# Benny44/QPALM

Hardware: AMD Instinct MI355X
Metric: QP solves/sec (batched random n=1000,m=2000); `value` = solve only, batch resident in HBM -- with qpalm_setup in the clock as the reference's run_time has it: `value_setup_plus_solve` (higher is better)
Workload: dtype f64

## Files before the change

### qpalm_amd/csrc/qpalm_capi.inc

```
#include <math.h>
#include <stdio.h>
#include <stdlib.h>
#include <string.h>
#include <sys/mman.h>

#include <algorithm>
#include <atomic>
#include <chrono>
#include <thread>
#include <string>
#include <vector>
#include <map>

#include "../../include/qpalm_gfx950.h"

#ifdef QP_TWO_INSTANCES
#define QP_INST(ns, kern) ns::kern
#else
#define QP_INST(ns, kern) kern
#define QP_T_SMALL QP_T
#define QP_LDS_SMALL 38912
#define QP_T_TINY QP_T
#define QP_LDS_TINY 22016
#define QP_TINY_PER_CU 7
// ... 57 lines not shown
  int lds_bytes;
  int max_slots;
  int update_rank_threshold;
  int narrow_rows;
  int place_panel_wave;
  int small_workgroups;
  int coop;
  int coop_workgroups;
  int coop_max_batch;
  int coop_rank_threshold;
  int queue_order;
  int coop_test_kill;
  int coop_graphs;
  int coop_updates;
  int sweep_ranks;
  int kkt_compact;
  int sequential_rank_sums;
  int linesearch_hbm;
  int sparse_gpw;
  int sparse_lds;
  int sparse_ordering;
  int sparse_factor;
  int sparse_coop;
  int sparse_kkt;
  int ld_align;
  void *mv_buf[5];
  size_t mv_cap[5];
};

enum { H_AP, H_AI, H_ATP, H_ATI, H_ATPERM, H_AINV, H_QP, H_QI, H_QFP, H_QFI, H_QFPERM, H_AX, H_QX, H_Q, H_BMIN, H_BMAX, H_COUNT };
// ... 44 lines not shown
  double *raw_bmax() { return raw_h.data() + (size_t)B * n + (size_t)B * m; }
  double *raw_d_q() const { return (double *)raw_d; }
  double *raw_d_bmin() const { return (double *)raw_d + (size_t)B * n; }
  double *raw_d_bmax() const { return (double *)raw_d + (size_t)B * n + (size_t)B * m; }
};
static void co_graphs_clear(qpg_batch *bt) {
  for (auto &g : bt->co_graphs) if (g.second.ready) RT_GRAPH_FREE(g.second.exec);
  bt->co_graphs.clear();
}

extern "C" int qpg_ctx_create(int device, qpg_ctx **out) {
  if (!out) return fail(QPG_ERR_INVALID, "qpg_ctx_create: out is NULL");
  std::string why;
  if (RT_DEVICE_INIT(device, why) != 0) return fail(QPG_ERR_NO_DEVICE, "qpg_ctx_create: " + why);
  qpg_ctx *c = new qpg_ctx();
  c->device = device; c->lds_bytes = QPG_LDS_DEFAULT; c->max_slots = 512; c->update_rank_threshold = -1; c->small_workgroups = 1; c->place_panel_wave = 0; c->narrow_rows = 1; c->coop = -1; c->coop_workgroups = 256; c->coop_max_batch = 4; c->coop_rank_threshold = -2; c->coop_updates = 2; c->coop_test_kill = 0; c->queue_order = 1; c->coop_graphs = 1; c->ld_align = 16; c->sweep_ranks = 16; c->kkt_compact = 1; c->sparse_factor = -1; c->sparse_kkt = 0; c->sparse_coop = 0; c->sparse_ordering = -1; c->sparse_lds = 1; c->sparse_gpw = 0; c->linesearch_hbm = 0; c->sequential_rank_sums = -1;
  for (int k = 0; k < 5; k++) { c->mv_buf[k] = nullptr; c->mv_cap[k] = 0; }
  *out = c;
  return api_ok();
}
extern "C" void qpg_ctx_destroy(qpg_ctx *ctx) {
  if (!ctx) return;
  for (int k = 0; k < 5; k++) if (ctx->mv_buf[k]) RT_FREE(ctx->mv_buf[k]);
  RT_RELEASE_STREAMS();
  delete ctx;
}
static int ctx_scratch(qpg_ctx *ctx, int k, size_t bytes, void **p) {
  if (bytes > ctx->mv_cap[k]) {
    if (ctx->mv_buf[k]) RT_FREE(ctx->mv_buf[k]);
    ctx->mv_buf[k] = nullptr; ctx->mv_cap[k] = 0;
    const size_t cap = align_up(bytes + bytes / 2, 4096);
// ... 7 lines not shown
  if (!ctx || !name) return fail(QPG_ERR_INVALID, "qpg_ctx_set_option: NULL");
  if (!strcmp(name, "lds_bytes")) { if (value < QPG_LDS_DEFAULT || value > 160 * 1024 - 8192) return fail(QPG_ERR_INVALID, "lds_bytes out of range"); ctx->lds_bytes = (int)value; }
  else if (!strcmp(name, "max_slots")) { if (value < 1) return fail(QPG_ERR_INVALID, "max_slots < 1"); ctx->max_slots = (int)value; }
  else if (!strcmp(name, "update_rank_threshold")) ctx->update_rank_threshold = (int)value;
  else if (!strcmp(name, "small_workgroups")) ctx->small_workgroups = (value >= 0 && value <= 3) ? (int)value : 1;
  else if (!strcmp(name, "place_panel_wave")) ctx->place_panel_wave = (value < 0 || value > 2) ? 2 : (int)value;
  else if (!strcmp(name, "narrow_rows")) ctx->narrow_rows = value ? 1 : 0;
  else if (!strcmp(name, "coop")) ctx->coop = (value < 0) ? -1 : (value ? 1 : 0);
  else if (!strcmp(name, "coop_rank_threshold")) ctx->coop_rank_threshold = (value < -1) ? -2 : (int)value;
  else if (!strcmp(name, "coop_updates")) ctx->coop_updates = (value >= 0 && value <= 2) ? (int)value : 2;
  else if (!strcmp(name, "coop_graphs")) ctx->coop_graphs = value ? 1 : 0;
  else if (!strcmp(name, "coop_test_kill")) ctx->coop_test_kill = (int)value;
  else if (!strcmp(name, "queue_order")) ctx->queue_order = value ? 1 : 0;
  else if (!strcmp(name, "sweep_ranks")) { if (value != 16 && value != 32) return fail(QPG_ERR_INVALID, "sweep_ranks must be 16 or 32"); ctx->sweep_ranks = (int)value; }
  else if (!strcmp(name, "kkt_compact")) ctx->kkt_compact = value ? 1 : 0;
  else if (!strcmp(name, "sparse_factor")) ctx->sparse_factor = (value < 0) ? -1 : (value ? 1 : 0);
  else if (!strcmp(name, "sparse_kkt")) ctx->sparse_kkt = value ? 1 : 0;
  else if (!strcmp(name, "sparse_coop")) { if (value != 0 && value != 1) return fail(QPG_ERR_INVALID, "sparse_coop must be 0 or 1"); ctx->sparse_coop = (int)value; }
  else if (!strcmp(name, "sequential_rank_sums")) ctx->sequential_rank_sums = (value < 0) ? -1 : (value ? 1 : 0);
  else if (!strcmp(name, "linesearch_hbm")) ctx->linesearch_hbm = (value < 0) ? 0 : (int)std::min<qpg_int>(value, 1 << 20);
  else if (!strcmp(name, "sparse_gpw")) ctx->sparse_gpw = (int)value;
  else if (!strcmp(name, "sparse_lds")) ctx->sparse_lds = (value < 0) ? 0 : (int)value;
  else if (!strcmp(name, "sparse_ordering")) ctx->sparse_ordering = (value < 0) ? -1 : (value ? 1 : 0);
  else if (!strcmp(name, "ld_align")) { if (value != 8 && value != 16 && value != 32) return fail(QPG_ERR_INVALID, "ld_align must be 8, 16 or 32"); ctx->ld_align = (int)value; }
  else if (!strcmp(name, "coop_max_batch")) { if (value < 1) return fail(QPG_ERR_INVALID, "coop_max_batch < 1"); ctx->coop_max_batch = (int)value; }
  else if (!strcmp(name, "coop_workgroups")) { if (value < 1 || value > 4096) return fail(QPG_ERR_INVALID, "coop_workgroups out of range"); ctx->coop_workgroups = (int)value; }
  else return fail(QPG_ERR_INVALID, std::string("unknown option ") + name);
  return api_ok();
}

// ... 731 lines not shown
  bt->raw_h.clear(); bt->raw_cur = 0;
  bt->val_maps_current = false;
  V.B = bt->B; V.n = bt->n; V.m = bt->m; V.ld = bt->ld; V.nnzA = bt->nnzA; V.nnzQ = bt->nnzQ; V.nnzQf = bt->nnzQf;
  V.ls_hbm = bt->ctx->linesearch_hbm; V.seq_mode = bt->ctx->sequential_rank_sums;
  V.nslots = bt->nslots; V.lds_bytes = bt->lds_bytes; V.update_rank_threshold = bt->ctx->update_rank_threshold; V.place_panel_wave = bt->ctx->place_panel_wave;
  V.ls_stride = bt->ls_stride;
  {
    size_t nnz_rows = 0, rows = 0;
    for (auto &hp : bt->probs) { nnz_rows += (size_t)hp.nzA; rows += (size_t)hp.m; }
    const size_t colbufs = (size_t)4 * (bt->threads / 64) * bt->n * sizeof(double);
    V.narrow_rows = (bt->ctx->narrow_rows && !bt->kkt && colbufs <= (size_t)bt->lds_bytes && nnz_rows <= 16 * std::max<size_t>(rows, 1)) ? 1 : 0;
  }
  V.wst_stride = (int)QPG_WST_STRIDE(bt->nfac);
  V.sweep_ranks = bt->ctx->sweep_ranks;
  V.kkt_compact = bt->ctx->kkt_compact;
  V.kkt = bt->kkt; V.nfac = bt->nfac;
  if (ensure_dual_slots(bt) != 0) return fail(QPG_ERR_ALLOC, "device allocation failed (LD_Q slots)");
  V.sparse = 0; V.sp_co_G = 0; V.sp_co_wv = nullptr;
  bt->sp_plan.clear();
  if (bt->sparse) {
    const int rcs = sparse_setup(bt);
    if (rcs != QPG_OK) return rcs;
    if (ensure_dual_slots(bt) != 0) return fail(QPG_ERR_ALLOC, "device allocation failed (LD_Q values of the sparse factor)");
  }
  const size_t B = bt->B, n = bt->n, m = bt->m;
  {
    char *const dev[H_COUNT] = {(char *)V.Ap, (char *)V.Ai, (char *)V.Atp, (char *)V.Ati, (char *)V.Atperm, (char *)V.Ainv, (char *)V.Qp, (char *)V.Qi,
                                (char *)V.Qfp, (char *)V.Qfi, (char *)V.Qfperm, (char *)V.Ax, (char *)V.Qx, (char *)V.q, (char *)V.bmin, (char *)V.bmax};
    for (int a = 0; a < H_COUNT; a++)
      if (bt->hper[a] && RT_MEMCPY_H2D_ASYNC(dev[a], bt->hslab + bt->hoff[a], B * bt->hper[a] * bt->helem[a], 0) != 0)
// ... 924 lines not shown
```

### qpalm_amd/csrc/qpalm_dense.h

```cpp
#ifndef QPALM_DENSE_H
#define QPALM_DENSE_H
#include <type_traits>

#ifdef QPALM_EMU
#define QP_FLAG_LOAD(p) (*(volatile int *)(p))
#define QP_FLAG_STORE(p, v) (*(volatile int *)(p) = (v))
#define QP_RELEASE_AGENT() do { } while (0)
#define QP_ACQUIRE_AGENT() do { } while (0)
#define QP_DRAIN_VMEM() do { } while (0)
#define QP_SLEEP() do { } while (0)
#define QP_WAVE_SYNC() emu_wave_sync()
#define QP_LDS_VBASE(p) (p)
#define QP_SCHED_BARRIER() do { } while (0)
#define QP_SETPRIO(p) do { } while (0)
#define QP_DRAIN_LDS() do { } while (0)
#else
#define QP_FLAG_LOAD(p) __hip_atomic_load((p), __ATOMIC_RELAXED, __HIP_MEMORY_SCOPE_AGENT)
#define QP_FLAG_STORE(p, v) __hip_atomic_store((p), (v), __ATOMIC_RELAXED, __HIP_MEMORY_SCOPE_AGENT)
#define QP_RELEASE_AGENT() __builtin_amdgcn_fence(__ATOMIC_RELEASE, "agent")
#define QP_ACQUIRE_AGENT() __builtin_amdgcn_fence(__ATOMIC_ACQUIRE, "agent")
#define QP_DRAIN_VMEM() asm volatile("s_waitcnt vmcnt(0)" ::: "memory")
#define QP_SLEEP() __builtin_amdgcn_s_sleep(2)
#define QP_SETPRIO(p) __builtin_amdgcn_s_setprio(p)
#define QP_DRAIN_LDS() asm volatile("s_waitcnt lgkmcnt(0)" ::: "memory")
// ... 265 lines not shown
};

#ifndef QP_NI_FGEMM
#define QP_NI_FGEMM QPNI
#endif
#ifndef QP_FKC
#define QP_FKC 32
#endif
#define QP_FAS 66
#ifndef QP_FST
#define QP_FST 4
#endif
struct FactorStage { double As[2][QP_FKC][QP_FAS]; };

template <int NTJ, int NCT>
QP_NI_FGEMM void factor_panel_update(double *L_, const double *Dg_, char *stage_, int n_, int ld_, int J_, int tbase_, int k0_, int k1_) {
  const int n = QP_UNIFORM(n_), ld = QP_UNIFORM(ld_), J = QP_UNIFORM(J_), tbase = QP_UNIFORM(tbase_), k0 = QP_UNIFORM(k0_), k1 = QP_UNIFORM(k1_);
  qp_gdouble *L = (qp_gdouble *)L_;
  const qp_gdouble *Dg = (const qp_gdouble *)Dg_;
  FactorStage QP_LDS_AS &F = *QP_LDS_ARG(FactorStage, stage_);
  const int tid = threadIdx.x, lane = tid & 63, wid = tid >> 6;
  const int l15 = lane & 15, l4 = lane >> 4;
  constexpr bool PAIR = (NTJ == 2);
  constexpr int NBW = 16 * NCT;
  const int rbase = (J / 16 + tbase) * 16 + wid * 16 * NTJ;
  auto rowof = [&](const int t, const int j) QP_ALWAYS_INLINE { return PAIR ? (rbase + 2 * j + t) : (rbase + j); };
  auto colof = [&](const int ct, const int i) QP_ALWAYS_INLINE { return J + NCT * i + ct; };
  qp_double4 acc[NTJ][NCT];
  const bool full = QP_UNIFORM((int)((rbase >= J + NBW) && (rbase + 16 * NTJ <= n) && (J + NBW <= n))) != 0;
  if (full) {
#pragma unroll
    for (int ct = 0; ct < NCT; ct++)
#pragma unroll
      for (int r = 0; r < 4; r++) {
        double v[NTJ];
        qp_load_rows<NTJ>(L + (size_t)colof(ct, l4 + 4 * r) * ld + rowof(0, l15), v);
// ... 82 lines not shown
    for (int t = 0; t < NTJ; t++) {
      const int row = rowof(t, l15);
      if (row < n) {
#pragma unroll
        for (int ct = 0; ct < NCT; ct++)
#pragma unroll
          for (int r = 0; r < 4; r++) {
            const int col = colof(ct, l4 + 4 * r);
            if (col < n && row >= col) L[(size_t)col * ld + row] = acc[t][ct][r];
          }
      }
    }
  }
}

#ifndef QP_NI_FROWS
#define QP_NI_FROWS QPNI
#endif
QP_NI_FROWS void factor_panel_rows(double *L_, char *lds_, const int n_, const int ld_, const int J_, const int jb_) {
  const int n = QP_UNIFORM(n_), ld = QP_UNIFORM(ld_), J = QP_UNIFORM(J_), jb = QP_UNIFORM(jb_);
  qp_gdouble *L = (qp_gdouble *)L_;
  FactorLds QP_LDS_AS &F = *QP_LDS_ARG(FactorLds, lds_);
  constexpr int NB = QP_FNB;
  auto rows = [&](auto full) QP_ALWAYS_INLINE {
    constexpr bool FULL = decltype(full)::value;
#pragma unroll 1
    for (int i = J + jb + threadIdx.x; i < n; i += QP_T) {
      qp_gdouble *base = L + (size_t)J * ld + i;
      double u[NB];
#pragma unroll
      for (int c = 0; c < NB; c++) u[c] = (FULL || c < jb) ? base[(size_t)c * ld] : 0.0;
#pragma unroll
      for (int c = 0; c < NB; c++) {
        if (FULL || c < jb) {
          double v = u[c];
#pragma unroll
          for (int c1 = 0; c1 < c; c1++) {
            v = QP_FMA(-u[c1], F.Ld[c][c1], v);
            if ((c1 & 7) == 7) QP_SCHED_BARRIER();
          }
          u[c] = v;
        }
        QP_SCHED_BARRIER();
      }
      int ld2 = ld;
      QP_OPAQUE(ld2);
#pragma unroll
      for (int c = 0; c < NB; c++)
        if (FULL || c < jb) base[(size_t)c * ld2] = u[c] * F.dv[c];
    }
  };
  if (jb == NB) rows(std::true_type()); else rows(std::false_type());
}

#ifndef QP_NI_FDIAG
#define QP_NI_FDIAG QPNI
#endif
QP_NI_FDIAG void factor_diag_block(char *lds_) {
  FactorLds QP_LDS_AS &F = *QP_LDS_ARG(FactorLds, lds_);
  constexpr int NB = QP_FNB;
  const int r = (int)(threadIdx.x & (NB - 1));
  double p[NB];
#pragma unroll
  for (int c = 0; c < NB; c++) p[c] = F.Ld[r][c];
#pragma unroll
  for (int c = 0; c < NB; c++) {
    const double dc = qp_readlane(p[c], c);
    const double lic = p[c] / dc;
#pragma unroll
    for (int c2 = c + 1; c2 < NB; c2++) {
      const double s = qp_readlane(p[c], c2);
      p[c2] = QP_FMA(-lic, s, p[c2]);
    }
    p[c] = lic;
    if (r == c && threadIdx.x < NB) { F.dv[c] = 1.0 / dc; F.dg[c] = dc; }
  }
  if (threadIdx.x < NB) {
#pragma unroll
    for (int c = 0; c < NB; c++) if (r > c) F.Ld[r][c] = p[c];
  }
}

template <int RPT>
#ifndef QP_NI_FACTOR
#define QP_NI_FACTOR QPNI
#endif
QP_NI_FACTOR void dense_factor(double *L_, double *Dg_, int n_, int ld_, char *lds_, int64_t *tdbg_) {
  const int n = QP_UNIFORM(n_), ld = QP_UNIFORM(ld_);
  int64_t QP_LDS_AS *tdbg = (int64_t QP_LDS_AS *)tdbg_;
  qp_gdouble *L = (qp_gdouble *)L_, *Dg = (qp_gdouble *)Dg_;
  FactorLds QP_LDS_AS &F = *QP_LDS_ARG(FactorLds, lds_);
  const int tid = threadIdx.x, lane = tid & 63, wid = tid >> 6;
  const int NB = QP_FNB;
  __syncthreads();
  long long tq0 = QP_CLOCK();
  for (int J = 0; J < n; J += NB) {
    const int jb = (n - J < NB) ? (n - J) : NB;
    {
      const bool super = (J % (2 * NB)) == 0;
      const int k0 = super ? 0 : J - NB, k1 = J;
      if (k1 > k0) {
        const int ntiles = (n - J + 15) / 16;
        char *stage = lds_ + ((sizeof(FactorLds) + 15) & ~(size_t)15);
        for (int tbase = 0; tbase < ntiles; tbase += QP_FNT * QP_NW) {
          const int rem = ntiles - tbase;
          const int ntj = (rem + QP_NW - 1) / QP_NW;
          if (super) {
            if (ntj <= 1) factor_panel_update<1, 4>(L_, Dg_, stage, n, ld, J, tbase, k0, k1);
            else factor_panel_update<2, 4>(L_, Dg_, stage, n, ld, J, tbase, k0, k1);
          } else {
            if (ntj <= 1) factor_panel_update<1, 2>(L_, Dg_, stage, n, ld, J, tbase, k0, k1);
            else factor_panel_update<2, 2>(L_, Dg_, stage, n, ld, J, tbase, k0, k1);
          }
        }
        if (tid == 0) {
          const long long npass = (ntiles + QP_FNT * QP_NW - 1) / (QP_FNT * QP_NW);
          tdbg[QPG_CNT_FACTOR_REREAD] += (long long)(n - J) * (k1 - k0) + npass * (super ? 2 * NB : NB) * (long long)(k1 - k0);
        }
      }
    }
    __syncthreads();
    if (tid == 0) { const long long tq1 = QP_CLOCK(); tdbg[4] += tq1 - tq0; tq0 = tq1; }
    for (int e = tid; e < NB * NB; e += QP_T) {
      const int c = e / NB, r = e % NB;
      F.Ld[r][c] = (r >= c && r < jb) ? L[(size_t)(J + c) * ld + (J + r)] : ((r == c) ? 1.0 : 0.0);
    }
    __syncthreads();
    if (wid == 0) factor_diag_block(lds_);
    __syncthreads();
    for (int e = tid; e < jb * jb; e += QP_T) {
      const int c = e / jb, r = e % jb;
      if (r > c) L[(size_t)(J + c) * ld + (J + r)] = F.Ld[r][c];
    }
    if (tid < jb) Dg[J + tid] = F.dg[tid];
    if (tid == 0) { const long long tq1 = QP_CLOCK(); tdbg[5] += tq1 - tq0; tq0 = tq1; }
    factor_panel_rows(L_, lds_, n, ld, J, jb);
    __syncthreads();
    if (tid == 0) { const long long tq1 = QP_CLOCK(); tdbg[6] += tq1 - tq0; tq0 = tq1; }
  }
  __syncthreads();
}

#define QP_SNB 32
#ifndef QP_SOLVE_FCH
#define QP_SOLVE_FCH 16
#endif
#ifndef QP_SOLVE_BU
#define QP_SOLVE_BU 4
#endif
struct SolveLds {
  double tile[2][QP_SNB][QP_SNB + 1];
  double part[QP_SNB];
};

// ... 1347 lines not shown
```

### qpalm_amd/csrc/qpalm_device.h

```cpp
#ifndef QPALM_DEVICE_H
#define QPALM_DEVICE_H

#include "qpalm_types.h"

#ifndef QP_T
#define QP_T 512
#endif
#define QP_NW (QP_T / 64)
#ifndef QP_KSEL
#define QP_KSEL(RPT) ((RPT) <= 2 ? 16 : 8)
#endif
#ifndef QP_K32
#ifdef QPALM_EMU
#define QP_K32(RPT) ((RPT) >= 1 && (RPT) <= 2)
#define QP_LDS_BUDGET QPG_LDS_DEFAULT
#else
#define QP_K32(RPT) (QP_T >= 512 && (RPT) >= 1 && (RPT) <= 2)
#define QP_LDS_BUDGET ((QP_T >= 512) ? QPG_LDS_DEFAULT : 38912)
#endif
#endif
#define QPD __device__ __forceinline__
#define QPN __device__ __forceinline__
#ifndef QP_PHASE_CALLS
#define QP_PHASE_CALLS 2
// ... 30 lines not shown
#endif

#ifdef QPALM_EMU
typedef emu_double4 qp_double4;
#define QP_MFMA_F64(a, b, c) emu_mfma_f64_16x16x4((a), (b), (c))
#define QP_DYN_LDS() (emu::dyn_lds())
#define QP_FMA(a, b, c) std::fma((a), (b), (c))
#define QP_SQRT(x) std::sqrt(x)
#define QP_CLOCK() ((long long)wall_clock64())
#define QP_UNIFORM(x) (x)
#define QP_UNIFORM_PTR(p) (p)
#define QP_OPAQUE(x) do { } while (0)
#define QP_OPAQUE_V(x) do { } while (0)
#define QP_FRESH_LANE(lane) (lane)
#define QP_CALL_BLOCK() 1
#define QP_ALWAYS_INLINE
#define QP_HW_CU_KEY() 0
#define QP_HW_SIMD() ((int)(threadIdx.x >> 6) & 3)
#else
typedef double qp_double4 __attribute__((ext_vector_type(4)));
#define QP_MFMA_F64(a, b, c) __builtin_amdgcn_mfma_f64_16x16x4f64((a), (b), (c), 0, 0, 0)
extern __shared__ __attribute__((aligned(16))) char qp_dyn_lds_[];
static __device__ __forceinline__ char *qp_dyn_lds_opaque_() {
  unsigned a = (unsigned)(size_t)(char __attribute__((address_space(3))) *)qp_dyn_lds_;
  asm volatile("" : "+s"(a));
  return (char *)(char __attribute__((address_space(3))) *)(size_t)a;
}
#define QP_DYN_LDS() (qp_dyn_lds_opaque_())
#define QP_FMA(a, b, c) fma((a), (b), (c))
#define QP_SQRT(x) sqrt(x)
// ... 1 lines not shown
#define QP_UNIFORM(x) __builtin_amdgcn_readfirstlane(x)
template <class P> static __device__ __forceinline__ P qp_uniform_ptr_(P p) {
  const unsigned long long a = (unsigned long long)p;
  const unsigned lo = (unsigned)__builtin_amdgcn_readfirstlane((int)(unsigned)a), hi = (unsigned)__builtin_amdgcn_readfirstlane((int)(unsigned)(a >> 32));
  return (P)(((unsigned long long)hi << 32) | lo);
}
#define QP_UNIFORM_PTR(p) qp_uniform_ptr_(p)
#define QP_OPAQUE(x) do { (x) = __builtin_amdgcn_readfirstlane(x); asm volatile("" : "+s"(x)); } while (0)
#define QP_OPAQUE_V(x) asm volatile("" : "+v"(x))
static __device__ __forceinline__ int qp_fresh_lane_() {
  int z = 0;
  asm volatile("s_mov_b32 %0, 0" : "=s"(z));
  return (int)__builtin_amdgcn_mbcnt_hi(~0u, __builtin_amdgcn_mbcnt_lo(~0u, (unsigned)z));
}
#define QP_FRESH_LANE(lane) qp_fresh_lane_()
static __device__ __forceinline__ int qp_opaque_true_() {
  int one;
  asm volatile("s_mov_b32 %0, 1" : "=s"(one));
  return one;
}
#define QP_CALL_BLOCK() qp_opaque_true_()
#define QP_ALWAYS_INLINE __attribute__((always_inline))
#define QP_HW_SIMD() ((int)__builtin_amdgcn_s_getreg((2 - 1) << 11 | 4 << 6 | 4))
#define QP_HW_CU_KEY() ((int)(__builtin_amdgcn_s_getreg((8 - 1) << 11 | 8 << 6 | 4) | (__builtin_amdgcn_s_getreg((4 - 1) << 11 | 0 << 6 | 20) << 8)))
#endif

QPD double qmax(double a, double b) { return (a > b) ? a : b; }
QPD double qmin(double a, double b) { return (a < b) ? a : b; }
QPD double qabs(double x) { return (x < 0) ? -x : x; }

// ... 191 lines not shown
```

### qpalm_amd/csrc/qpalm_iter.h

```cpp
#ifndef QPALM_ITER_H
#define QPALM_ITER_H
#ifndef QP_NOFUSE
#define QP_NOFUSE 0
#endif

#define QP_KIND_NEWTON 0
#define QP_KIND_OUTER 1
#define QP_KIND_FORCED 2
#define QP_KIND_TERMINATED 3

QPD int qp_prox(const qpg_settings &st, const qpg_scalars &s) { return (st.proximal != 0 || s.nc_flag != 0) ? 1 : 0; }
QPD double qp_gamma_init(const qpg_settings &st, const qpg_scalars &s) { return s.nc_flag ? s.nc_gamma : st.gamma_init; }
QPD double qp_gamma_max(const qpg_settings &st, const qpg_scalars &s) { return s.nc_flag ? s.nc_gamma : st.gamma_max; }

struct IterShared {
  QpShared S;
  qpg_scalars s;
  int kind, action, nL, pos;
  double a0, b0;
  double scan_a[QP_NW], scan_b[QP_NW];
};

struct QpArrays {
  const qpg_view *V; int b, n, m;
// ... 187 lines not shown
    vs[2] += t * t;
  }
  block_reduce<0, 3>(I.S, vm, vs);
  const double f = 0.5 * vs[0] + vs[1], dist2 = vs[2];
  const double sig = qmax(1e-4, qmin(st.sigma_init * qmax(1, qabs(f)) / qmax(1, 0.5 * dist2), 1e4));
  const double ssig = QP_SQRT(sig), sinv = 1.0 / sig;
  for (int i = tid; i < m; i += QP_T) {
    a.sigma()[i] = sig; a.sigma_inv()[i] = sinv; a.sqrt_sigma()[i] = ssig; a.At_scale()[i] = ssig;
    for (int k = a.Atp()[i]; k < a.Atp()[i + 1]; k++) a.Atss()[k] = a.Atx()[k] * ssig;
  }
  if (tid == 0) { I.s.sqrt_sigma_max = QP_SQRT(st.sigma_max); I.s.initialized = 1; }
  __syncthreads();
}

template <int RPT>
QPN void dev_factor(const qpg_view &V, int n, double *L, double *Dg, char *lds, int64_t *tdbg) { dense_factor<RPT>(L, Dg, n, V.ld, lds, tdbg); }
template <int RPT>
QPN void dev_updown(const qpg_view &V, int b, int n, double *L, double *Dg, double *Wst, const int *up, int n_up,
                    const int *dn, int n_dn, QpShared &S, char *lds, int64_t *tdbg, double *fs = nullptr, int pre_jmin = -1) {
  const int *Atp = V.Atp + (size_t)b * (V.m + 1), *Ati = V.Ati + (size_t)b * V.nnzA;
  const double *Atss = V.Atss + (size_t)b * V.nnzA;
  __syncthreads();
  if (threadIdx.x == 0) S.seq_ranks = qp_pivot_mode(V, b);
  __syncthreads();
  if constexpr (RPT == 0) dense_updown_big<16>(Atp, Ati, Atss, n, V.ld, L, Dg, Wst, up, n_up, dn, n_dn, &S, lds, tdbg, pre_jmin);
  else if constexpr (QP_K32(RPT)) {
    const int nr = n_up + n_dn;
    int n32 = 0;
    if (V.sweep_ranks >= 32 && pre_jmin < 0 && nr > 16) n32 = (nr % 32 > 16 || nr % 32 == 0) ? nr : nr - nr % 32;
    if (n32 > 0) dense_updown<1, 32>(Atp, Ati, Atss, n, V.ld, L, Dg, Wst, up, n_up, dn, n_dn, &S, lds, tdbg, -1, (n32 == nr) ? fs : nullptr, 0, n32);
    if (n32 < nr) dense_updown<RPT, QP_KSEL(RPT)>(Atp, Ati, Atss, n, V.ld, L, Dg, Wst, up, n_up, dn, n_dn, &S, lds, tdbg, pre_jmin, fs, n32, nr - n32);
// ... 663 lines not shown
    }
    if (V.offload && !resume && !V.kkt && (la == 1 || la == 3 || la == 7 || (kind == QP_KIND_NEWTON && la == 0) || (V.offload >= 2 && (la == 2 || la == 4)))) {
      if (kind == QP_KIND_NEWTON && la != 7) {
        for (int j = tid; j < n; j += QP_T) a.d()[j] = a.dphi()[j] * -1;
      }
      __syncthreads();
      if (tid == 0) {
        I.s.pend_stage = 1; I.s.pend_la = (la == 1 || la == 3 || la == 7 || la == 2 || la == 4) ? la : 0; I.s.pend_action = action; I.s.pend_kind = kind;
        I.s.pend_nchange = (la == 4) ? n_sig : nchange; I.s.pend_gam = gam;
      }
      __syncthreads();
      break;
    }
    const long long t0 = QP_CLOCK();
    double gersh_ub = 0.0;
    if constexpr (SPARSE) {
      const SpArrays SP = sp_arrays(V, b, slot, Dg, lds);
      if (resume) {
        if (la == 7) {
          SpArrays SQ = SP; SQ.Lx = LQ; SQ.Dg = DgQ;
          const double dobj = dev_dual_objective_sp(V, a, b, SQ, I);
          if (tid == 0) { I.s.dual_objective = dobj; I.s.dual_pending = 0; }
          __syncthreads();
          continue;
        }
      } else
      if (la == 2) {
        sp_updown(V, b, n, SP, a.enter(), I.s.nb_enter, a.leave(), I.s.nb_leave);
        if (V.offload && kind == QP_KIND_NEWTON) {
          for (int j = tid; j < n; j += QP_T) a.d()[j] = a.dphi()[j] * -1;
// ... 16 lines not shown
        continue;
      }
    } else
    if (resume) {
      if (la == 7) {
        const double dobj = dev_dual_objective(V, a, b, LQ, DgQ, I, lds);
        if (tid == 0) { I.s.dual_objective = dobj; I.s.dual_pending = 0; }
        __syncthreads();
        continue;
      }
    } else
    if (la == 1 || la == 3 || la == 5 || la == 7) {
      double *Lt = (la == 7) ? LQ : L, *Dt = (la == 7) ? DgQ : Dg;
      gersh_ub = form_schur(V, b, n, Lt, la == 5, la == 1 || la == 5, (la == 1 || la == 3) && (prox != 0), gam, I.S, lds);
      if (tid == 0) I.s.ticks_dbg[3] += QP_CLOCK() - t0;
      if (la != 5) dev_factor<RPT>(V, n, Lt, Dt, lds, I.s.ticks_dbg);
      if (dual_init) {
        const double dobj = dev_dual_objective(V, a, b, LQ, DgQ, I, lds);
        if (tid == 0) { I.s.dual_objective = dobj; I.s.dual_pending = 0; }
        __syncthreads();
        continue;
      }
    } else if (la == 8) {
      kkt_newton<RPT>(&V, b, L, Dg, Wst, &I, lds, action, I.s.nb_enter, I.s.nb_leave, QP_KKT_SOLVE | QP_KKT_REFINE);
    } else if (la == 2 || la == 4) {
      const int n_up = (la == 2) ? I.s.nb_enter : n_sig, n_dn = (la == 2) ? I.s.nb_leave : 0;
      double *fs = nullptr;
      constexpr bool FUSED = (RPT > 0) && !QP_NOFUSE;
      if (FUSED && la == 2 && !V.offload) {
        for (int j = tid; j < n; j += QP_T) a.d()[j] = a.dphi()[j] * -1;
        fs = a.d();
// ... 10 lines not shown
    }
    const long long t1 = QP_CLOCK();
    QP_OPAQUE(a.b);
    if (la == 4) {
      dev_update_sigma_post(a, I, n_sig);
      if (tid == 0) { I.s.n_sweeps = (int)I.s.ticks_dbg[QPG_CNT_SWEEPS]; I.s.ticks_update += t1 - t0; }
    } else if (la == 5 || la == 6) dev_boost_gamma_apply(V, a, I, gersh_ub);
    if (kind == QP_KIND_NEWTON) {
      if constexpr (SPARSE) {
        if (!V.kkt && !resume) {
          for (int j = tid; j < n; j += QP_T) a.d()[j] = a.dphi()[j] * -1;
          sp_solve(n, sp_arrays(V, b, slot, Dg, lds), a.d());
        }
      } else
      if (!V.kkt && !resume) {
        const bool fused = (RPT > 0) && !QP_NOFUSE && (action == 2) && !V.offload;
        if (!fused) for (int j = tid; j < n; j += QP_T) a.d()[j] = a.dphi()[j] * -1;
        __syncthreads();
        dense_solve(L, Dg, n, V.ld, a.d(), lds, V.lds_bytes, I.s.ticks_dbg, fused ? 2 : 0);
      }
      const long long t2 = QP_CLOCK();
      for (int i = tid; i < m; i += QP_T) a.active_old()[i] = a.active()[i];
      if (tid == 0) {
        I.s.reset_newton = 0;
        I.s.kkt_first = 0;
        if (action == 1) { I.s.n_refactor++; I.s.ticks_factor += t1 - t0; }
        if (action == 3) { I.s.n_factor_Q++; I.s.ticks_factor += t1 - t0; }
        if (action == 2) { if (!V.kkt) I.s.n_rank1 += nchange; I.s.n_sweeps = (int)I.s.ticks_dbg[QPG_CNT_SWEEPS]; I.s.ticks_update += t1 - t0; }
        I.s.n_solve++; I.s.ticks_solve += t2 - t1;
        if (!V.kkt && (RPT > 0) && !QP_NOFUSE && action == 2 && (SPARSE || !V.offload)) I.s.n_fused_solve++;
        I.s.last_fact = action;
      }
      QP_OPAQUE(a.b);
      const double tau = dev_linesearch(V, a, I, lds);
      const long long t3 = QP_CLOCK();
      QP_OPAQUE(a.b);
      {
        const int gs = QP_UNIFORM(I.s.guard_spent);
        const double ge = I.s.eta, gb = I.s.beta;
        const bool bad = !(qabs(ge) <= 1.7976931348623157e308) || !(qabs(gb) <= 1.7976931348623157e308);
        const int what = ((action == 0 || action == 2 || gs == 2) && gs != 1 && bad) ? ((gs == 2) ? 2 : 1) : ((gs == 2) ? 3 : 0);
        const int w = QP_UNIFORM(what);
        if (w != 0) {
          __syncthreads();
          if (tid == 0) {
// ... 51 lines not shown
```

### qpalm_amd/csrc/qpalm_kkt.h

```cpp
#ifndef QPALM_KKT_H
#define QPALM_KKT_H

QPD void kkt_form(const qpg_view &V, const QpArrays &a, int b, double *L, double gamma, int prox) {
  const int n = a.n, m = a.m, np = n + m, ld = V.ld, tid = threadIdx.x;
  int *state = V.kkt_state + (size_t)b * V.m;
  __syncthreads();
  for (int j = 0; j < np; j++)
    for (int i = j + tid; i < np; i += QP_T) L[(size_t)j * ld + i] = 0.0;
  __syncthreads();
  for (int j = tid; j < n; j += QP_T) {
    for (int k = a.Qp()[j]; k < a.Qp()[j + 1]; k++) { const int i = a.Qi()[k]; if (i >= j) L[(size_t)j * ld + i] += a.Qx()[k]; }
    if (prox) L[(size_t)j * ld + j] += 1.0 / gamma;
  }
  for (int k = tid; k < m; k += QP_T) {
    const int p = n + k, e0 = a.Atp()[k], e1 = a.Atp()[k + 1];
    if (a.active()[k]) {
      state[k] = 1;
      for (int e = e0; e < e1; e++) L[(size_t)a.Ati()[e] * ld + p] = a.Atx()[e];
      L[(size_t)p * ld + p] = (e1 > e0) ? -a.sigma_inv()[k] : 1.0;
    } else { state[k] = 0; L[(size_t)p * ld + p] = 1.0; }
  }
  __syncthreads();
}

// ... 136 lines not shown
  const qpg_view &V = *Vp;
  IterShared &I = *Ip;
  const int b = QP_UNIFORM(b_), action = QP_UNIFORM(action_), ne = QP_UNIFORM(ne_), nl = QP_UNIFORM(nl_), flags = QP_UNIFORM(flags_);
  const QpArrays a = qp_arrays(V, b);
  const qpg_settings &st = *V.settings;
  const int n = a.n, m = a.m, np = n + m, ld = V.ld, tid = threadIdx.x, lane = tid & 63, wid = tid >> 6, prox = qp_prox(st, I.s);
  const double gamma = I.s.gamma;
  const size_t sk = (size_t)V.n + V.m;
  double *sol = V.kkt_sol + (size_t)b * sk, *rhs = V.kkt_rhs + (size_t)b * sk, *z = V.kkt_tmp + (size_t)b * sk;
  int *state = V.kkt_state + (size_t)b * V.m;
  int *list = V.kkt_list + (size_t)b * V.m;
  const bool can_compact = V.kkt_compact && ((size_t)QP_NW * np * sizeof(double) + (size_t)m * sizeof(int) <= (size_t)V.lds_bytes);
  int kna = QP_UNIFORM(I.s.kkt_na);
  if (action == 1 && can_compact) {
    kna = kkt_form_compact(V, a, b, L, gamma, prox, I, list);
    dense_factor<RPT>(L, Dg, n + kna, ld, lds, I.s.ticks_dbg);
  } else {
    if (kna >= 0 && (action == 2 || action == 5)) { kkt_expand(V, a, L, Dg, kna, list, lds); kna = -1; }
    if (action == 1 || action == 3) { kkt_form(V, a, b, L, gamma, prox); kna = -1; }
    if (action == 1 || action == 4) { dense_factor<RPT>(L, Dg, np, ld, lds, I.s.ticks_dbg); kna = -1; }
  }
  __syncthreads();
  if (tid == 0) I.s.kkt_na = kna;
  __syncthreads();
  if (action == 2) {
    for (int e = 0; e < ne + nl; e++) {
      const bool add = e < ne;
      const int k = QP_UNIFORM(add ? a.enter()[e] : a.leave()[e - ne]), p = n + k;
      __syncthreads();
      int up;
      if (add) {
        for (int j = tid; j < np; j += QP_T) z[j] = 0.0;
        __syncthreads();
        for (int q = a.Atp()[k] + tid; q < a.Atp()[k + 1]; q += QP_T) z[a.Ati()[q]] = a.Atx()[q];
        __syncthreads();
// ... 76 lines not shown
```

### qpalm_amd/csrc/qpalm_types.h

```cpp
#ifndef QPALM_TYPES_H_GFX950
#define QPALM_TYPES_H_GFX950

#include <stdint.h>

#define QPG_SOLVED 1
#define QPG_DUAL_TERMINATED 2
#define QPG_MAX_ITER_REACHED (-2)
#define QPG_PRIMAL_INFEASIBLE (-3)
#define QPG_DUAL_INFEASIBLE (-4)
#define QPG_TIME_LIMIT_REACHED (-5)
#define QPG_UNSOLVED (-10)
#define QPG_ERROR 0
#define QPG_INFTY 1e20

typedef struct {
  int64_t max_iter, inner_max_iter;
  double eps_abs, eps_rel, eps_abs_in, eps_rel_in, rho, eps_prim_inf, eps_dual_inf, theta, delta, sigma_max,
      sigma_init;
  int64_t proximal;
  double gamma_init, gamma_upd, gamma_max;
  int64_t scaling, nonconvex, verbose, print_iter, warm_start, reset_newton_iter, enable_dual_termination;
  double dual_objective_limit, time_limit;
  int64_t ordering, factorization_method, max_rank_update;
  double max_rank_update_fraction;
// ... 24 lines not shown
  int32_t pend_stage, pend_la, pend_action, pend_kind, pend_nchange;
  int32_t seq_hint;
  int32_t kkt_na;
  double pend_gam;
  int64_t pend_clock;
  int32_t guard_redo, n_guard_refactor, guard_spent, guard_pad;
  int32_t dual_pending, kkt_first;
  int32_t n_refactor, n_factor_Q, n_sweeps, n_rank1, n_solve, n_sigma_updates, n_boost_gamma, n_fused_solve;
  int64_t ticks_total, ticks_factor, ticks_update, ticks_solve, ticks_linesearch, ticks_resid;
  int64_t ticks_dbg[QPG_NDBG];
} qpg_scalars;

typedef struct {
  int32_t B, n, m, ld, nnzA, nnzQ, nnzQf, nslots, lds_bytes, update_rank_threshold, ls_stride, wst_stride, place_panel_wave, narrow_rows;
  int32_t offload, sweep_ranks;
  int32_t kkt_compact, kkt_pad;
  int32_t kkt, nfac;
  int32_t *Ap, *Ai, *Atp, *Ati, *Atperm, *Ainv, *Qp, *Qi, *Qfp, *Qfi, *Qfperm;
  double *Ax, *Atx, *Atss, *Qx, *Qfx;
  double *q, *bmin, *bmax, *c0;
  double *x, *y, *Axv, *Qxv, *Aty, *x_prev, *x0;
  double *sigma, *sigma_inv, *sqrt_sigma, *At_scale;
  double *Axys, *z, *pri_res, *pri_res_in, *yh, *Atyh, *df, *dphi, *dphi_prev, *d, *Qd, *Ad;
  double *delta_y, *delta_x, *temp_n, *temp_m;
  double *D, *Dinv, *E, *Einv;
  double *ls_key;
  int32_t *ls_idx;
  double *ls_delta, *ls_alpha;
  int32_t *active, *active_old, *enter, *leave;
  double *sol_x, *sol_y;
  double *L;
// ... 43 lines not shown
```

Measured before the change: 5363.

## Fuse forward substitution into dense LDL factorization for Newton refactors

During a full dense factorization in the Newton step, the right-hand side is kept in LDS and the forward triangular solve is done alongside the factorization. The diagonal block applies its unit-lower solve to the panel's entries, and the panel-row pass updates the remaining entries as L columns are produced. The later dense_solve then skips its forward phase, which saves one extra pass over L in HBM. This costs extra LDS for an n-length vector, adds a fit check, and inlines previously noinline helpers, which may change register pressure.

```diff
diff --git a/qpalm_amd/csrc/qpalm_capi.inc b/qpalm_amd/csrc/qpalm_capi.inc
--- a/qpalm_amd/csrc/qpalm_capi.inc
+++ b/qpalm_amd/csrc/qpalm_capi.inc
@@ -95,6 +95,7 @@
   int coop_graphs;
   int coop_updates;
   int sweep_ranks;
+  int factor_fused_solve;
   int kkt_compact;
   int sequential_rank_sums;
   int linesearch_hbm;
@@ -169,7 +170,7 @@
   std::string why;
   if (RT_DEVICE_INIT(device, why) != 0) return fail(QPG_ERR_NO_DEVICE, "qpg_ctx_create: " + why);
   qpg_ctx *c = new qpg_ctx();
-  c->device = device; c->lds_bytes = QPG_LDS_DEFAULT; c->max_slots = 512; c->update_rank_threshold = -1; c->small_workgroups = 1; c->place_panel_wave = 0; c->narrow_rows = 1; c->coop = -1; c->coop_workgroups = 256; c->coop_max_batch = 4; c->coop_rank_threshold = -2; c->coop_updates = 2; c->coop_test_kill = 0; c->queue_order = 1; c->coop_graphs = 1; c->ld_align = 16; c->sweep_ranks = 16; c->kkt_compact = 1; c->sparse_factor = -1; c->sparse_kkt = 0; c->sparse_coop = 0; c->sparse_ordering = -1; c->sparse_lds = 1; c->sparse_gpw = 0; c->linesearch_hbm = 0; c->sequential_rank_sums = -1;
+  c->device = device; c->lds_bytes = QPG_LDS_DEFAULT; c->max_slots = 512; c->update_rank_threshold = -1; c->small_workgroups = 1; c->place_panel_wave = 0; c->narrow_rows = 1; c->coop = -1; c->coop_workgroups = 256; c->coop_max_batch = 4; c->coop_rank_threshold = -2; c->coop_updates = 2; c->coop_test_kill = 0; c->queue_order = 1; c->coop_graphs = 1; c->ld_align = 16; c->sweep_ranks = 16; c->kkt_compact = 1; c->factor_fused_solve = 1; c->sparse_factor = -1; c->sparse_kkt = 0; c->sparse_coop = 0; c->sparse_ordering = -1; c->sparse_lds = 1; c->sparse_gpw = 0; c->linesearch_hbm = 0; c->sequential_rank_sums = -1;
   for (int k = 0; k < 5; k++) { c->mv_buf[k] = nullptr; c->mv_cap[k] = 0; }
   *out = c;
   return api_ok();
@@ -207,6 +208,7 @@
   else if (!strcmp(name, "queue_order")) ctx->queue_order = value ? 1 : 0;
   else if (!strcmp(name, "sweep_ranks")) { if (value != 16 && value != 32) return fail(QPG_ERR_INVALID, "sweep_ranks must be 16 or 32"); ctx->sweep_ranks = (int)value; }
   else if (!strcmp(name, "kkt_compact")) ctx->kkt_compact = value ? 1 : 0;
+  else if (!strcmp(name, "factor_fused_solve")) ctx->factor_fused_solve = value ? 1 : 0;
   else if (!strcmp(name, "sparse_factor")) ctx->sparse_factor = (value < 0) ? -1 : (value ? 1 : 0);
   else if (!strcmp(name, "sparse_kkt")) ctx->sparse_kkt = value ? 1 : 0;
   else if (!strcmp(name, "sparse_coop")) { if (value != 0 && value != 1) return fail(QPG_ERR_INVALID, "sparse_coop must be 0 or 1"); ctx->sparse_coop = (int)value; }
@@ -968,6 +970,7 @@
   V.wst_stride = (int)QPG_WST_STRIDE(bt->nfac);
   V.sweep_ranks = bt->ctx->sweep_ranks;
   V.kkt_compact = bt->ctx->kkt_compact;
+  V.factor_fused_solve = bt->ctx->factor_fused_solve;
   V.kkt = bt->kkt; V.nfac = bt->nfac;
   if (ensure_dual_slots(bt) != 0) return fail(QPG_ERR_ALLOC, "device allocation failed (LD_Q slots)");
   V.sparse = 0; V.sp_co_G = 0; V.sp_co_wv = nullptr;
diff --git a/qpalm_amd/csrc/qpalm_dense.h b/qpalm_amd/csrc/qpalm_dense.h
--- a/qpalm_amd/csrc/qpalm_dense.h
+++ b/qpalm_amd/csrc/qpalm_dense.h
@@ -303,12 +303,12 @@
 struct FactorStage { double As[2][QP_FKC][QP_FAS]; };
 
 template <int NTJ, int NCT>
-QP_NI_FGEMM void factor_panel_update(double *L_, const double *Dg_, char *stage_, int n_, int ld_, int J_, int tbase_, int k0_, int k1_) {
+QPD void factor_panel_update_body(double *L_, const double *Dg_, char *stage_, int n_, int ld_, int J_, int tbase_, int k0_, int k1_) {
   const int n = QP_UNIFORM(n_), ld = QP_UNIFORM(ld_), J = QP_UNIFORM(J_), tbase = QP_UNIFORM(tbase_), k0 = QP_UNIFORM(k0_), k1 = QP_UNIFORM(k1_);
   qp_gdouble *L = (qp_gdouble *)L_;
   const qp_gdouble *Dg = (const qp_gdouble *)Dg_;
   FactorStage QP_LDS_AS &F = *QP_LDS_ARG(FactorStage, stage_);
-  const int tid = threadIdx.x, lane = tid & 63, wid = tid >> 6;
+  const int tid = QP_FRESH_TID(), lane = tid & 63, wid = tid >> 6;
   const int l15 = lane & 15, l4 = lane >> 4;
   constexpr bool PAIR = (NTJ == 2);
   constexpr int NBW = 16 * NCT;
@@ -421,18 +421,27 @@
   }
 }
 
+#define QP_FACTOR_YS_OFF (((sizeof(FactorLds) + 15) & ~(size_t)15) + sizeof(FactorStage))
+QPD bool factor_solve_fits(const int n, const int lds_bytes) { return QP_FACTOR_YS_OFF + (size_t)n * sizeof(double) <= (size_t)lds_bytes; }
+
+template <int NTJ, int NCT>
+QP_NI_FGEMM void factor_panel_update(double *L_, const double *Dg_, char *stage_, int n_, int ld_, int J_, int tbase_, int k0_, int k1_) {
+  factor_panel_update_body<NTJ, NCT>(L_, Dg_, stage_, n_, ld_, J_, tbase_, k0_, k1_);
+}
+
 #ifndef QP_NI_FROWS
-#define QP_NI_FROWS QPNI
-#endif
-QP_NI_FROWS void factor_panel_rows(double *L_, char *lds_, const int n_, const int ld_, const int J_, const int jb_) {
+#define QP_NI_FROWS QPD
+#endif
+QP_NI_FROWS void factor_panel_rows(double *L_, char *lds_, const int n_, const int ld_, const int J_, const int jb_, const int fuse_ = 0) {
   const int n = QP_UNIFORM(n_), ld = QP_UNIFORM(ld_), J = QP_UNIFORM(J_), jb = QP_UNIFORM(jb_);
   qp_gdouble *L = (qp_gdouble *)L_;
   FactorLds QP_LDS_AS &F = *QP_LDS_ARG(FactorLds, lds_);
+  double QP_LDS_AS *ys = QP_LDS_ARG(double, lds_ + QP_FACTOR_YS_OFF);
   constexpr int NB = QP_FNB;
-  auto rows = [&](auto full) QP_ALWAYS_INLINE {
-    constexpr bool FULL = decltype(full)::value;
+  auto rows = [&](auto full, auto fused) QP_ALWAYS_INLINE {
+    constexpr bool FULL = decltype(full)::value, FUSE = decltype(fused)::value;
 #pragma unroll 1
-    for (int i = J + jb + threadIdx.x; i < n; i += QP_T) {
+    for (int i = J + jb + QP_FRESH_TID(); i < n; i += QP_T) {
       qp_gdouble *base = L + (size_t)J * ld + i;
       double u[NB];
 #pragma unroll
@@ -452,21 +461,34 @@
       }
       int ld2 = ld;
       QP_OPAQUE(ld2);
-#pragma unroll
-      for (int c = 0; c < NB; c++)
-        if (FULL || c < jb) base[(size_t)c * ld2] = u[c] * F.dv[c];
+      if (FUSE) {
+        double acc = ys[i];
+#pragma unroll
+        for (int c = 0; c < NB; c++)
+          if (FULL || c < jb) {
+            const double l = u[c] * F.dv[c];
+            base[(size_t)c * ld2] = l;
+            acc = QP_FMA(-l, ys[J + c], acc);
+          }
+        ys[i] = acc;
+      } else {
+#pragma unroll
+        for (int c = 0; c < NB; c++)
+          if (FULL || c < jb) base[(size_t)c * ld2] = u[c] * F.dv[c];
+      }
     }
   };
-  if (jb == NB) rows(std::true_type()); else rows(std::false_type());
+  if (QP_UNIFORM(fuse_) != 0) { if (jb == NB) rows(std::true_type(), std::true_type()); else rows(std::false_type(), std::true_type()); }
+  else { if (jb == NB) rows(std::true_type(), std::false_type()); else rows(std::false_type(), std::false_type()); }
 }
 
 #ifndef QP_NI_FDIAG
 #define QP_NI_FDIAG QPNI
 #endif
-QP_NI_FDIAG void factor_diag_block(char *lds_) {
+QPD void factor_diag_block_body(char *lds_, const int fuse = 0, const int J = 0, const int jb = 0) {
   FactorLds QP_LDS_AS &F = *QP_LDS_ARG(FactorLds, lds_);
   constexpr int NB = QP_FNB;
-  const int r = (int)(threadIdx.x & (NB - 1));
+  const int tx = QP_FRESH_TID(), r = tx & (NB - 1);
   double p[NB];
 #pragma unroll
   for (int c = 0; c < NB; c++) p[c] = F.Ld[r][c];
@@ -480,29 +502,50 @@
       p[c2] = QP_FMA(-lic, s, p[c2]);
     }
     p[c] = lic;
-    if (r == c && threadIdx.x < NB) { F.dv[c] = 1.0 / dc; F.dg[c] = dc; }
-  }
-  if (threadIdx.x < NB) {
+    if (r == c && tx < NB) { F.dv[c] = 1.0 / dc; F.dg[c] = dc; }
+  }
+  if (tx < NB) {
 #pragma unroll
     for (int c = 0; c < NB; c++) if (r > c) F.Ld[r][c] = p[c];
   }
-}
-
-template <int RPT>
+  if (fuse) {
+    double QP_LDS_AS *ys = QP_LDS_ARG(double, lds_ + QP_FACTOR_YS_OFF);
+    const int lane = tx;
+    double v = (lane < jb) ? ys[J + lane] : 0.0;
+#pragma unroll
+    for (int c = 0; c < NB; c++) {
+      const double yc = qp_readlane(v, c);
+      const double l = (r > c && r < jb) ? p[c] : 0.0;
+      v = QP_FMA(-l, yc, v);
+    }
+    if (lane < jb) ys[J + lane] = v;
+  }
+}
+
+QP_NI_FDIAG void factor_diag_block(char *lds_) { factor_diag_block_body(lds_); }
+
 #ifndef QP_NI_FACTOR
 #define QP_NI_FACTOR QPNI
 #endif
-QP_NI_FACTOR void dense_factor(double *L_, double *Dg_, int n_, int ld_, char *lds_, int64_t *tdbg_) {
+QP_NI_FACTOR void dense_factor(double *La_, double *Dga_, int n_, int ld_, char *ldsa_, int64_t *tdbga_, const double *fb_ = nullptr, double *fs_ = nullptr) {
   const int n = QP_UNIFORM(n_), ld = QP_UNIFORM(ld_);
+  double *L_ = QP_UNIFORM_PTR(La_), *Dg_ = QP_UNIFORM_PTR(Dga_);
+  char *lds_ = QP_UNIFORM_PTR(ldsa_);
+  int64_t *tdbg_ = QP_UNIFORM_PTR(tdbga_);
+  qp_gdouble *fs = (qp_gdouble *)QP_UNIFORM_PTR(fs_);
+  const qp_gdouble *fb = (const qp_gdouble *)QP_UNIFORM_PTR(fb_);
+  const int fuse = (fs != nullptr) ? 1 : 0;
+  double QP_LDS_AS *ys = QP_LDS_ARG(double, lds_ + QP_FACTOR_YS_OFF);
   int64_t QP_LDS_AS *tdbg = (int64_t QP_LDS_AS *)tdbg_;
   qp_gdouble *L = (qp_gdouble *)L_, *Dg = (qp_gdouble *)Dg_;
   FactorLds QP_LDS_AS &F = *QP_LDS_ARG(FactorLds, lds_);
-  const int tid = threadIdx.x, lane = tid & 63, wid = tid >> 6;
   const int NB = QP_FNB;
   __syncthreads();
+  if (fuse) for (int i = QP_FRESH_TID(); i < n; i += QP_T) ys[i] = fb[i] * -1;
   long long tq0 = QP_CLOCK();
   for (int J = 0; J < n; J += NB) {
     const int jb = (n - J < NB) ? (n - J) : NB;
+    int tid = QP_FRESH_TID();
     {
       const bool super = (J % (2 * NB)) == 0;
       const int k0 = super ? 0 : J - NB, k1 = J;
@@ -513,11 +556,11 @@
           const int rem = ntiles - tbase;
           const int ntj = (rem + QP_NW - 1) / QP_NW;
           if (super) {
-            if (ntj <= 1) factor_panel_update<1, 4>(L_, Dg_, stage, n, ld, J, tbase, k0, k1);
-            else factor_panel_update<2, 4>(L_, Dg_, stage, n, ld, J, tbase, k0, k1);
+            if (ntj <= 1) factor_panel_update_body<1, 4>(L_, Dg_, stage, n, ld, J, tbase, k0, k1);
+            else factor_panel_update_body<2, 4>(L_, Dg_, stage, n, ld, J, tbase, k0, k1);
           } else {
-            if (ntj <= 1) factor_panel_update<1, 2>(L_, Dg_, stage, n, ld, J, tbase, k0, k1);
-            else factor_panel_update<2, 2>(L_, Dg_, stage, n, ld, J, tbase, k0, k1);
+            if (ntj <= 1) factor_panel_update_body<1, 2>(L_, Dg_, stage, n, ld, J, tbase, k0, k1);
+            else factor_panel_update_body<2, 2>(L_, Dg_, stage, n, ld, J, tbase, k0, k1);
           }
         }
         if (tid == 0) {
@@ -528,23 +571,26 @@
     }
     __syncthreads();
     if (tid == 0) { const long long tq1 = QP_CLOCK(); tdbg[4] += tq1 - tq0; tq0 = tq1; }
+    tid = QP_FRESH_TID();
     for (int e = tid; e < NB * NB; e += QP_T) {
       const int c = e / NB, r = e % NB;
       F.Ld[r][c] = (r >= c && r < jb) ? L[(size_t)(J + c) * ld + (J + r)] : ((r == c) ? 1.0 : 0.0);
     }
     __syncthreads();
-    if (wid == 0) factor_diag_block(lds_);
+    if ((tid >> 6) == 0) factor_diag_block_body(lds_, fuse, J, jb);
     __syncthreads();
+    tid = QP_FRESH_TID();
     for (int e = tid; e < jb * jb; e += QP_T) {
       const int c = e / jb, r = e % jb;
       if (r > c) L[(size_t)(J + c) * ld + (J + r)] = F.Ld[r][c];
     }
     if (tid < jb) Dg[J + tid] = F.dg[tid];
     if (tid == 0) { const long long tq1 = QP_CLOCK(); tdbg[5] += tq1 - tq0; tq0 = tq1; }
-    factor_panel_rows(L_, lds_, n, ld, J, jb);
+    factor_panel_rows(L_, lds_, n, ld, J, jb, fuse);
     __syncthreads();
-    if (tid == 0) { const long long tq1 = QP_CLOCK(); tdbg[6] += tq1 - tq0; tq0 = tq1; }
-  }
+    if (QP_FRESH_TID() == 0) { const long long tq1 = QP_CLOCK(); tdbg[6] += tq1 - tq0; tq0 = tq1; }
+  }
+  if (fuse) for (int i = QP_FRESH_TID(); i < n; i += QP_T) fs[i] = ys[i];
   __syncthreads();
 }
 
diff --git a/qpalm_amd/csrc/qpalm_device.h b/qpalm_amd/csrc/qpalm_device.h
--- a/qpalm_amd/csrc/qpalm_device.h
+++ b/qpalm_amd/csrc/qpalm_device.h
@@ -68,6 +68,7 @@
 #define QP_OPAQUE_V(x) do { } while (0)
 #define QP_FRESH_LANE(lane) (lane)
 #define QP_CALL_BLOCK() 1
+#define QP_FRESH_TID() ((int)threadIdx.x)
 #define QP_ALWAYS_INLINE
 #define QP_HW_CU_KEY() 0
 #define QP_HW_SIMD() ((int)(threadIdx.x >> 6) & 3)
@@ -99,6 +100,12 @@
   return (int)__builtin_amdgcn_mbcnt_hi(~0u, __builtin_amdgcn_mbcnt_lo(~0u, (unsigned)z));
 }
 #define QP_FRESH_LANE(lane) qp_fresh_lane_()
+static __device__ __forceinline__ int qp_fresh_tid_() {
+  int t = (int)threadIdx.x;
+  asm volatile("" : "+v"(t));
+  return t & 1023;
+}
+#define QP_FRESH_TID() qp_fresh_tid_()
 static __device__ __forceinline__ int qp_opaque_true_() {
   int one;
   asm volatile("s_mov_b32 %0, 1" : "=s"(one));
diff --git a/qpalm_amd/csrc/qpalm_iter.h b/qpalm_amd/csrc/qpalm_iter.h
--- a/qpalm_amd/csrc/qpalm_iter.h
+++ b/qpalm_amd/csrc/qpalm_iter.h
@@ -225,7 +225,7 @@
 }
 
 template <int RPT>
-QPN void dev_factor(const qpg_view &V, int n, double *L, double *Dg, char *lds, int64_t *tdbg) { dense_factor<RPT>(L, Dg, n, V.ld, lds, tdbg); }
+QPN void dev_factor(const qpg_view &V, int n, double *L, double *Dg, char *lds, int64_t *tdbg, const double *fb = nullptr, double *fs = nullptr) { dense_factor(L, Dg, n, V.ld, lds, tdbg, fb, fs); }
 template <int RPT>
 QPN void dev_updown(const qpg_view &V, int b, int n, double *L, double *Dg, double *Wst, const int *up, int n_up,
                     const int *dn, int n_dn, QpShared &S, char *lds, int64_t *tdbg, double *fs = nullptr, int pre_jmin = -1) {
@@ -919,6 +919,7 @@
     }
     const long long t0 = QP_CLOCK();
     double gersh_ub = 0.0;
+    int factor_fused = 0;
     if constexpr (SPARSE) {
       const SpArrays SP = sp_arrays(V, b, slot, Dg, lds);
       if (resume) {
@@ -965,7 +966,8 @@
       double *Lt = (la == 7) ? LQ : L, *Dt = (la == 7) ? DgQ : Dg;
       gersh_ub = form_schur(V, b, n, Lt, la == 5, la == 1 || la == 5, (la == 1 || la == 3) && (prox != 0), gam, I.S, lds);
       if (tid == 0) I.s.ticks_dbg[3] += QP_CLOCK() - t0;
-      if (la != 5) dev_factor<RPT>(V, n, Lt, Dt, lds, I.s.ticks_dbg);
+      factor_fused = QP_UNIFORM((int)(!SPARSE && (la == 1 || la == 3) && kind == QP_KIND_NEWTON && !V.kkt && !V.offload && V.factor_fused_solve && factor_solve_fits(n, V.lds_bytes)));
+      if (la != 5) dev_factor<RPT>(V, n, Lt, Dt, lds, I.s.ticks_dbg, factor_fused ? a.dphi() : nullptr, factor_fused ? a.d() : nullptr);
       if (dual_init) {
         const double dobj = dev_dual_objective(V, a, b, LQ, DgQ, I, lds);
         if (tid == 0) { I.s.dual_objective = dobj; I.s.dual_pending = 0; }
@@ -1006,7 +1008,7 @@
         }
       } else
       if (!V.kkt && !resume) {
-        const bool fused = (RPT > 0) && !QP_NOFUSE && (action == 2) && !V.offload;
+        const bool fused = ((RPT > 0) && !QP_NOFUSE && (action == 2) && !V.offload) || factor_fused;
         if (!fused) for (int j = tid; j < n; j += QP_T) a.d()[j] = a.dphi()[j] * -1;
         __syncthreads();
         dense_solve(L, Dg, n, V.ld, a.d(), lds, V.lds_bytes, I.s.ticks_dbg, fused ? 2 : 0);
@@ -1020,7 +1022,7 @@
         if (action == 3) { I.s.n_factor_Q++; I.s.ticks_factor += t1 - t0; }
         if (action == 2) { if (!V.kkt) I.s.n_rank1 += nchange; I.s.n_sweeps = (int)I.s.ticks_dbg[QPG_CNT_SWEEPS]; I.s.ticks_update += t1 - t0; }
         I.s.n_solve++; I.s.ticks_solve += t2 - t1;
-        if (!V.kkt && (RPT > 0) && !QP_NOFUSE && action == 2 && (SPARSE || !V.offload)) I.s.n_fused_solve++;
+        if ((!V.kkt && (RPT > 0) && !QP_NOFUSE && action == 2 && (SPARSE || !V.offload)) || factor_fused) I.s.n_fused_solve++;
         I.s.last_fact = action;
       }
       QP_OPAQUE(a.b);
diff --git a/qpalm_amd/csrc/qpalm_kkt.h b/qpalm_amd/csrc/qpalm_kkt.h
--- a/qpalm_amd/csrc/qpalm_kkt.h
+++ b/qpalm_amd/csrc/qpalm_kkt.h
@@ -174,11 +174,11 @@
   int kna = QP_UNIFORM(I.s.kkt_na);
   if (action == 1 && can_compact) {
     kna = kkt_form_compact(V, a, b, L, gamma, prox, I, list);
-    dense_factor<RPT>(L, Dg, n + kna, ld, lds, I.s.ticks_dbg);
+    dense_factor(L, Dg, n + kna, ld, lds, I.s.ticks_dbg);
   } else {
     if (kna >= 0 && (action == 2 || action == 5)) { kkt_expand(V, a, L, Dg, kna, list, lds); kna = -1; }
     if (action == 1 || action == 3) { kkt_form(V, a, b, L, gamma, prox); kna = -1; }
-    if (action == 1 || action == 4) { dense_factor<RPT>(L, Dg, np, ld, lds, I.s.ticks_dbg); kna = -1; }
+    if (action == 1 || action == 4) { dense_factor(L, Dg, np, ld, lds, I.s.ticks_dbg); kna = -1; }
   }
   __syncthreads();
   if (tid == 0) I.s.kkt_na = kna;
diff --git a/qpalm_amd/csrc/qpalm_types.h b/qpalm_amd/csrc/qpalm_types.h
--- a/qpalm_amd/csrc/qpalm_types.h
+++ b/qpalm_amd/csrc/qpalm_types.h
@@ -62,7 +62,7 @@
 typedef struct {
   int32_t B, n, m, ld, nnzA, nnzQ, nnzQf, nslots, lds_bytes, update_rank_threshold, ls_stride, wst_stride, place_panel_wave, narrow_rows;
   int32_t offload, sweep_ranks;
-  int32_t kkt_compact, kkt_pad;
+  int32_t kkt_compact, factor_fused_solve;
   int32_t kkt, nfac;
   int32_t *Ap, *Ai, *Atp, *Ati, *Atperm, *Ainv, *Qp, *Qi, *Qfp, *Qfi, *Qfperm;
   double *Ax, *Atx, *Atss, *Qx, *Qfx;
```

Result: faster. 5502, median of 6 (+2.6%).
